# bowang-lab/BioReason

Hardware: AMD Instinct MI355X
Metric: GRPO samples/sec (NT-500M+Qwen3-1.7B, DNA 2x1024, prompt 2180, gen 256) (higher is better)
Workload: dtype bf16

## Files before the change

bioreason_amd/csrc/k_decgemm.hip:

```cpp
#include "bra_decgemm.h"
#include "bra_api_internal.h"

namespace bra {

#define BRA_DG2_HEAD_PARAMS const bf16_t* h_x, const bf16_t* h_W, const bf16_t* h_res, const float* h_ss_in, int h_ldx, int h_ldres, int h_M, int h_N, \
                            int h_K, int h_nss_in
#define BRA_DG2_HEAD_ARGS(g) (g).x, (g).W, (g).res, (g).ss_in, (int)(g).ldx, (int)(g).ldres, (g).M, (g).N, (g).K, (g).nss_in
template <int MODE, int NORM, int ACT, int OUTF32, int NW, int NL, int WIDE = 0, int PK = 0, int FAST = 0, int F8 = 0>
__global__ __launch_bounds__(NW * 64) void dec_gemm2_kernel(BRA_DG2_HEAD_PARAMS, DecGemm2Args g0) {
    DecGemm2Args g = g0;
    g.x = h_x; g.W = h_W; g.res = h_res; g.ss_in = h_ss_in; g.ldx = h_ldx; g.ldres = h_ldres; g.M = h_M; g.N = h_N; g.K = h_K; g.nss_in = h_nss_in;
    constexpr bool W32 = WIDE >= 2;
    static_assert(WIDE != 3 || (!FAST && NORM == 0), "32 rows, multi-round: not the fast form, no folded norm");
    static_assert(!WIDE || (MODE == 0 && NORM != 1), "wide rows: 16-column tiles, statistics applied in the epilogue");
    static_assert(!FAST || (PK && NORM != 1), "fast form: packed weights, folded norm or none");
    static_assert(!F8 || (FAST && NL % 2 == 0 && NW != 16 && !WIDE), "fp8 weights: fast form, two k-steps per 16-byte request");
    static_assert(WIDE != 2 || !F8, "32 rows: bf16 weights");
    constexpr int NLW = F8 ? NL / 2 : NL;
    constexpr int NH = W32 ? 2 : 1;
    constexpr int NBUF = (W32 && NW == 16) ? 1 : 2;
    __shared__ float red[NBUF][NH * NW][64][4];
    constexpr int KS = MODE ? 64 : 32;
    constexpr int NCOL = MODE ? 8 : 16;
    const int tid = (int)threadIdx.x, lane = tid & 63, wave = tid >> 6;
    const int fr = lane & 15, fq = lane >> 4;
    if (!FAST) dg2_stamp(g, 0);
    const int nsteps = FAST ? NW * NL : g.K / KS;
    const int ntiles = (g.N + NCOL - 1) / NCOL;
    const int lrow = MODE ? (fr & 7) : fr;
    const int koff = MODE ? ((fr >> 3) * 32 + fq * 8) : fq * 8;
    const int xr = lrow < g.M ? lrow : g.M - 1;
    const bf16_t* xp = FAST ? g.x + (dg2_mul24(xr, (int)g.ldx) + (unsigned)koff) : g.x + (long)xr * g.ldx + koff;
    auto x2_ptr = [&]() -> const bf16_t* {
        const int xr2 = lrow + 16 < g.M ? lrow + 16 : g.M - 1;
        return FAST ? g.x + (dg2_mul24(xr2, (int)g.ldx) + (unsigned)koff) : g.x + (long)xr2 * g.ldx + koff;
    };
    auto second_half = [&]() -> DecGemm2Args {
        DecGemm2Args g2 = g;
        g2.M = g.M - 16;
        if (g.res) g2.res = g.res + 16 * g.ldres;
        g2.out = OUTF32 ? (void*)((float*)g.out + 16 * g.ldo) : (void*)((bf16_t*)g.out + 16 * g.ldo);
        if (g.ss_out) g2.ss_out = g.ss_out + 16 * (long)g.nss_out;
        return g2;
    };
    const u32x4 zero4 = {0u, 0u, 0u, 0u};
    const int rounds = FAST ? 1 : (nsteps + NW * NL - 1) / (NW * NL);
    int tile = (int)blockIdx.x;
    int rn = tile * NCOL + lrow; rn = rn < g.N ? rn : g.N - 1;
    const bf16_t* wp = FAST ? g.W : g.W + (long)rn * g.ldw + koff;

    const int em = fr < g.M ? fr : g.M - 1;
    int en = tile * NCOL + 4 * fq; en = en + 3 < g.N ? en : (g.N >= 4 ? g.N - 4 : 0);
    u32x2 resv = {0u, 0u}, resv2 = {0u, 0u};
    if (!FAST && !ACT && !OUTF32 && g.res) resv = ld8(g.res + (long)em * g.ldres + en);
    auto em2_row = [&]() -> int { return fr + 16 < g.M ? fr : g.M - 17; };

    const int per = NORM ? g.nss_in >> 3 : 0;
    f32x4 pv[8];
    __shared__ float rs_lds[W32 ? 32 : (WIDE ? 16 : 8)];
    if (NORM == 1) {
        const float* pp = g.ss_in + (long)(lane >> 3) * g.nss_in + (lane & 7) * per;
#pragma unroll
        for (int i = 0; i < 8; ++i) pv[i] = *reinterpret_cast<const f32x4*>(pp + (4 * i < per ? 4 * i : 0));
    }
    float rstd = 1.f;

    if (WIDE != 3 && rounds == 1) {
        int st[NL];
#pragma unroll
        for (int u = 0; u < NL; ++u)
            st[u] = PK ? wave * NL + u
                             : (MODE ? wave + NW * u : 2 * (wave + NW * (u >> 1)) + (u & 1));
        long so[NL];
#pragma unroll
        for (int u = 0; u < NL; ++u) so[u] = FAST ? (long)(u * KS) : (long)(st[u] < nsteps ? st[u] : nsteps - 1) * KS;
        if (FAST) xp += (unsigned)(wave * (NL * KS));
        constexpr bool X2LATE = W32 && NW == 16;
        u32x4 w0[NLW], w1[NLW], x[NL], nv[NL], x2[(W32 && !X2LATE) ? NL : 1];
        f32x4 sc0 = {1.f, 1.f, 1.f, 1.f}, sc1 = sc0;
#pragma unroll
        for (int u = 0; u < NL; ++u) x[u] = ld16(xp + so[u]);
        if (NORM == 1) {
#pragma unroll
            for (int u = 0; u < NL; ++u) nv[u] = ld16(g.nw + koff + so[u]);
        }
        long wo[NLW];
#pragma unroll
        for (int u = 0; u < NLW; ++u) wo[u] = FAST ? (long)(u * 512) : (PK ? (long)(st[u] < nsteps ? st[u] : nsteps - 1) * 512 : so[u]);
        const unsigned wlane = (unsigned)(wave * (NLW * 512) + lane * 8);
        auto scale_of = [&](int t) -> f32x4 {
            return *reinterpret_cast<const f32x4*>(g.wscale + (unsigned)(t * NCOL + ((4 * fq) & (NCOL - 1))));
        };
        auto tile_base = [&](int t) -> const bf16_t* {
            if (FAST) return g.W + (long)t * (NW * NLW * 512) + wlane;
            if (PK) return g.W + (long)t * nsteps * 512 + lane * 8;
            int rnn = t * NCOL + lrow; rnn = rnn < g.N ? rnn : g.N - 1;
            return g.W + (long)rnn * g.ldw + koff;
        };
        wp = tile_base(tile);
#pragma unroll
        for (int u = 0; u < NLW; ++u) {
            w0[u] = ld16_nt(wp + wo[u]);
            if (W32 && u == 0) sched_fence();
        }
        const bf16_t* xp2 = xp;
        if constexpr (W32) {
            sched_fence();
            xp2 = x2_ptr();
            if (FAST) xp2 += (unsigned)(wave * (NL * KS));
            if constexpr (!X2LATE) {
#pragma unroll
                for (int u = 0; u < NL; ++u) x2[u] = ld16(xp2 + so[u]);
            }
            if (!FAST && !ACT && !OUTF32 && g.res) resv2 = ld8(g.res + (long)(em2_row() + 16) * g.ldres + en);
        }
        if (F8) {
            sched_fence();
            sc0 = scale_of(tile);
        }
        if (FAST && !ACT && !OUTF32) {
            const bf16_t* rp = g.res ? g.res : g.x;
            const unsigned ro = g.res ? dg2_mul24(em, (int)g.ldres) + (unsigned)en : 0u;
            resv = ld8(rp + ro);
            if (W32) resv2 = ld8(rp + (g.res ? dg2_mul24(em2_row() + 16, (int)g.ldres) + (unsigned)en : 0u));
        }
        sched_fence();
        if (!FAST) dg2_stamp(g, 1);
        constexpr int NPASS = WIDE == 1 ? 2 : 1;
        f32x4 sq[NPASS][8];
        const int swave = W32 ? 4 : 1, sbase = W32 ? 8 * wave : 0;
        if (NORM == 2 && wave < swave) {
#pragma unroll
            for (int pass = 0; pass < NPASS; ++pass) {
                const int srow = (lane >> 3) + 8 * pass + sbase;
                const int sr = srow < g.M ? srow : g.M - 1;
                const float* pp = FAST ? g.ss_in + (dg2_mul24(sr, g.nss_in) + (unsigned)((lane & 7) * per))
                                       : g.ss_in + (long)sr * g.nss_in + (lane & 7) * per;
#pragma unroll
                for (int i = 0; i < 8; ++i) sq[pass][i] = *reinterpret_cast<const f32x4*>(pp + (4 * i < per ? 4 * i : 0));
            }
#pragma unroll
            for (int pass = 0; pass < NPASS; ++pass)
#pragma unroll
                for (int i = 0; i < 8; ++i) reg_fence(sq[pass][i]);
        }
        auto fold_stats = [&]() {
#pragma unroll
            for (int pass = 0; pass < NPASS; ++pass) {
                const int srow = (lane >> 3) + 8 * pass + sbase;
                const float rs = dg2_fold_rstd(sq[pass], per, g.inv_K, g.eps);
                if ((lane & 7) == 0) rs_lds[srow] = rs;
            }
        };
        if (NORM == 1) {
#pragma unroll
            for (int i = 0; i < 8; ++i) reg_fence(pv[i]);
            float s = 0.f;
#pragma unroll
            for (int i = 0; i < 8; ++i) s += 4 * i < per ? (pv[i][0] + pv[i][1]) + (pv[i][2] + pv[i][3]) : 0.f;
            s += wave_shfl_xor(s, 1); s += wave_shfl_xor(s, 2); s += wave_shfl_xor(s, 4);
            rstd = rsqrtf(wave_shfl(s, xr * 8) / (float)g.K + g.eps);
#pragma unroll
            for (int u = 0; u < NL; ++u) {
                float xf[8], nf[8];
                unpack8(x[u], xf); unpack8(nv[u], nf);
#pragma unroll
                for (int i = 0; i < 8; ++i) xf[i] = nf[i] * round_bf(xf[i] * rstd);
                x[u] = pack8(xf);
            }
        }
#pragma unroll
        for (int u = 0; u < NL; ++u) if (!FAST && st[u] >= nsteps) x[u] = zero4;
        if constexpr (W32 && !X2LATE) {
#pragma unroll
            for (int u = 0; u < NL; ++u) if (!FAST && st[u] >= nsteps) x2[u] = zero4;
        }
        const int G = (int)gridDim.x;
        const int nmine = (ntiles - tile + G - 1) / G;
        auto issue = [&](u32x4 (&wn)[NLW], f32x4& scn, int t) {
            const bf16_t* wpn = tile_base(t);
#pragma unroll
            for (int u = 0; u < NLW; ++u) wn[u] = ld16_nt(wpn + wo[u]);
            if (F8) scn = scale_of(t);
        };
        auto compute = [&](u32x4 (&wc)[NLW], const f32x4& scc, int t, int it) {
            f32x4 acc = {0.f, 0.f, 0.f, 0.f};
            if constexpr (F8 != 0) {
#pragma unroll
                for (int u = 0; u < NLW; ++u) {
                    acc = mfma_16x16x32(f8x8_to_bf16x8(wc[u].x, wc[u].y), x[2 * u], acc);
                    acc = mfma_16x16x32(f8x8_to_bf16x8(wc[u].z, wc[u].w), x[2 * u + 1], acc);
                }
            } else {
#pragma unroll
                for (int u = 0; u < NL; ++u) acc = mfma_16x16x32(wc[u], x[u], acc);
            }
            f32x4 acc2 = {0.f, 0.f, 0.f, 0.f};
            if constexpr (X2LATE) {
                sched_fence();
#pragma unroll
                for (int u = 0; u < NL; ++u) x[u] = ld16(xp2 + so[u]);
#pragma unroll
                for (int u = 0; u < NL; ++u) if (!FAST && st[u] >= nsteps) x[u] = zero4;
#pragma unroll
                for (int u = 0; u < NL; ++u) acc2 = mfma_16x16x32(wc[u], x[u], acc2);
            } else if constexpr (W32) {
#pragma unroll
                for (int u = 0; u < NL; ++u) acc2 = mfma_16x16x32(wc[u], x2[u], acc2);
            }
            if (NORM == 2 && it == 0 && wave < swave) fold_stats();
            float (*slab)[64][4] = red[NBUF == 2 ? it & 1 : 0];
#pragma unroll
            for (int r = 0; r < 4; ++r) slab[wave][lane][r] = acc[r];
            if constexpr (W32) {
#pragma unroll
                for (int r = 0; r < 4; ++r) slab[NW + wave][lane][r] = acc2[r];
            }
            if (!FAST && it == 0) dg2_stamp(g, 2);
            __syncthreads();
            if (!FAST && it == 0) dg2_stamp(g, 3);
            if (wave == it % NW) {
                float v[4];
                dg2_reduce<NW>(slab, lane, v);
                if (NORM == 2) {
                    const int mrow = MODE ? (fr & 7) : fr;
                    const float rsf = rs_lds[mrow < g.M ? mrow : g.M - 1];
#pragma unroll
                    for (int r = 0; r < 4; ++r) v[r] *= rsf;
                }
                if (F8) {
#pragma unroll
                    for (int r = 0; r < 4; ++r) v[r] *= scc[r];
                }
                dg2_epilogue<MODE, ACT, OUTF32, PK>(g, v, t, lane, it == 0, resv);
            }
            if constexpr (W32) {
                if (wave == (it + 1) % NW) {
                    float v[4];
                    dg2_reduce<NW>(slab + NW, lane, v);
                    if (NORM == 2) {
                        const float rsf = rs_lds[16 + em2_row()];
#pragma unroll
                        for (int r = 0; r < 4; ++r) v[r] *= rsf;
                    }
                    const DecGemm2Args g2 = second_half();
                    dg2_epilogue<MODE, ACT, OUTF32, PK>(g2, v, t, lane, it == 0, resv2);
                }
            }
            if (!FAST && it == 0) dg2_stamp(g, 4);
        };
        if (NW == 16) {
            compute(w0, sc0, tile, 0);
            return;
        }
        int it = 0;
        for (; it + 2 < nmine; it += 2) {
            issue(w1, sc1, tile + (it + 1) * G); compute(w0, sc0, tile + it * G, it);
            issue(w0, sc0, tile + (it + 2) * G); compute(w1, sc1, tile + (it + 1) * G, it + 1);
        }
        if (nmine - it == 2) {
            issue(w1, sc1, tile + (it + 1) * G); compute(w0, sc0, tile + it * G, it);
            compute(w1, sc1, tile + (it + 1) * G, it + 1);
        } else {
            compute(w0, sc0, tile + it * G, it);
        }
        return;
    }

    if constexpr (WIDE == 2) return;
    constexpr bool X2LATE_MR = W32 && NW == 16;
    for (int it = 0; tile < ntiles; ++it, tile += (int)gridDim.x) {
        rn = tile * NCOL + lrow; rn = rn < g.N ? rn : g.N - 1;
        wp = g.W + (long)rn * g.ldw + koff;
        f32x4 acc = {0.f, 0.f, 0.f, 0.f}, acc2 = acc;
        for (int rd = 0; rd < rounds; ++rd) {
            const int base = rd * NW * NL;
            int st[NL];
#pragma unroll
            for (int u = 0; u < NL; ++u) st[u] = base + (MODE ? wave + NW * u : 2 * (wave + NW * (u >> 1)) + (u & 1));
            u32x4 w[NL], x[NL], nv[NL], x2[(W32 && !X2LATE_MR) ? NL : 1];
            const bf16_t* wpk = g.W + ((long)tile * nsteps * 64 + lane) * 8;
#pragma unroll
            for (int u = 0; u < NL; ++u) {
                const int sc = st[u] < nsteps ? st[u] : nsteps - 1;
                w[u] = PK ? ld16_nt(wpk + (long)sc * 512) : ld16_nt(wp + (long)sc * KS);
            }
#pragma unroll
            for (int u = 0; u < NL; ++u) { const int sc = st[u] < nsteps ? st[u] : nsteps - 1; x[u] = ld16(xp + (long)sc * KS); }
            const bf16_t* xp2 = xp;
            if constexpr (W32) {
                sched_fence();
                xp2 = x2_ptr();
                if (it == 0 && rd == 0 && !ACT && !OUTF32 && g.res) resv2 = ld8(g.res + (long)(em2_row() + 16) * g.ldres + en);
                if constexpr (!X2LATE_MR) {
#pragma unroll
                    for (int u = 0; u < NL; ++u) { const int sc = st[u] < nsteps ? st[u] : nsteps - 1; x2[u] = ld16(xp2 + (long)sc * KS); }
                }
            }
            if (NORM == 1) {
#pragma unroll
                for (int u = 0; u < NL; ++u) { const int sc = st[u] < nsteps ? st[u] : nsteps - 1; nv[u] = ld16(g.nw + koff + (long)sc * KS); }
                if (it == 0 && rd == 0) {
                    float s = 0.f;
#pragma unroll
                    for (int i = 0; i < 8; ++i) s += 4 * i < per ? (pv[i][0] + pv[i][1]) + (pv[i][2] + pv[i][3]) : 0.f;
                    s += wave_shfl_xor(s, 1); s += wave_shfl_xor(s, 2); s += wave_shfl_xor(s, 4);
                    rstd = rsqrtf(wave_shfl(s, xr * 8) / (float)g.K + g.eps);
                }
#pragma unroll
                for (int u = 0; u < NL; ++u) {
                    float xf[8], nf[8];
                    unpack8(x[u], xf); unpack8(nv[u], nf);
#pragma unroll
                    for (int i = 0; i < 8; ++i) xf[i] = nf[i] * round_bf(xf[i] * rstd);
                    x[u] = pack8(xf);
                }
            }
#pragma unroll
            for (int u = 0; u < NL; ++u) acc = mfma_16x16x32(st[u] < nsteps ? w[u] : zero4, x[u], acc);
            if constexpr (X2LATE_MR) {
                sched_fence();
#pragma unroll
                for (int u = 0; u < NL; ++u) { const int sc = st[u] < nsteps ? st[u] : nsteps - 1; x[u] = ld16(xp2 + (long)sc * KS); }
#pragma unroll
                for (int u = 0; u < NL; ++u) acc2 = mfma_16x16x32(st[u] < nsteps ? w[u] : zero4, x[u], acc2);
            } else if constexpr (W32) {
#pragma unroll
                for (int u = 0; u < NL; ++u) acc2 = mfma_16x16x32(st[u] < nsteps ? w[u] : zero4, x2[u], acc2);
            }
        }
        float (*slab)[64][4] = red[NBUF == 2 ? it & 1 : 0];
#pragma unroll
        for (int r = 0; r < 4; ++r) slab[wave][lane][r] = acc[r];
        if constexpr (W32) {
#pragma unroll
            for (int r = 0; r < 4; ++r) slab[NW + wave][lane][r] = acc2[r];
        }
        __syncthreads();
        if (wave == it % NW) {
            float v[4];
#pragma unroll
            for (int r = 0; r < 4; ++r) {
                float s = 0.f;
#pragma unroll
                for (int wv = 0; wv < NW; ++wv) s += slab[wv][lane][r];
                v[r] = s;
            }
            dg2_epilogue<MODE, ACT, OUTF32>(g, v, tile, lane, it == 0, resv);
        }
        if constexpr (W32) {
            if (wave == (it + 1) % NW) {
                float v[4];
#pragma unroll
                for (int r = 0; r < 4; ++r) {
                    float s = 0.f;
#pragma unroll
                    for (int wv = 0; wv < NW; ++wv) s += slab[NW + wv][lane][r];
                    v[r] = s;
                }
                const DecGemm2Args g2 = second_half();
                dg2_epilogue<MODE, ACT, OUTF32>(g2, v, tile, lane, it == 0, resv2);
            }
            if (NBUF == 1) __syncthreads();
        }
    }
}

__global__ __launch_bounds__(256) void row_sumsq_kernel(const bf16_t* x, long ldx, int K, float* ss, int nss) {
    __shared__ float part[4];
    const int r = (int)blockIdx.x, tid = (int)threadIdx.x;
    float s = 0.f;
    for (int j = tid; j < K / 8; j += 256) {
        float f[8];
        unpack8(ld16(x + (long)r * ldx + j * 8), f);
#pragma unroll
        for (int i = 0; i < 8; ++i) s += f[i] * f[i];
    }
    s = wave_sum<64>(s);
    if ((tid & 63) == 0) part[tid >> 6] = s;
    __syncthreads();
    for (int j = tid; j < nss; j += 256) ss[(long)r * nss + j] = j == 0 ? (part[0] + part[1]) + (part[2] + part[3]) : 0.f;
}

template <int MODE>
__global__ __launch_bounds__(256) void dec_pack_kernel(const bf16_t* W, long ldw, int N, int K, const bf16_t* nw, bf16_t* out) {
    constexpr int KS = MODE ? 64 : 32, NCOL = MODE ? 8 : 16;
    const int nsteps = K / KS;
    const long nchunk = (long)(N / NCOL) * nsteps * 64;
    const long c = (long)blockIdx.x * 256 + threadIdx.x;
    if (c >= nchunk) return;
    const int lane = (int)(c & 63);
    const long ts = c >> 6;
    const int step = (int)(ts % nsteps), tile = (int)(ts / nsteps);
    const int fr = lane & 15, fq = lane >> 4;
    const int row = tile * NCOL + (MODE ? (fr & 7) : fr);
    const int col = step * KS + (MODE ? ((fr >> 3) * 32 + fq * 8) : fq * 8);
    u32x4 v = ld16(W + (long)row * ldw + col);
    if (nw) {
        float f[8], s[8];
        unpack8(v, f); unpack8(ld16(nw + col), s);
#pragma unroll
        for (int i = 0; i < 8; ++i) f[i] *= s[i];
        v = pack8(f);
    }
    st16(out + c * 8, v);
}

__global__ __launch_bounds__(256) void dec_rowscale_fp8_kernel(const bf16_t* W, long ldw, int N, int K, const bf16_t* nw, float* scale) {
    const int row = (int)blockIdx.x * 4 + ((int)threadIdx.x >> 6), lane = (int)threadIdx.x & 63;
    if (row >= N) return;
    float mx = 0.f;
    for (int j = lane; j < K / 8; j += 64) {
        float f[8], s[8];
        unpack8(ld16(W + (long)row * ldw + j * 8), f);
        if (nw) { unpack8(ld16(nw + j * 8), s);
#pragma unroll
            for (int i = 0; i < 8; ++i) f[i] *= s[i]; }
#pragma unroll
        for (int i = 0; i < 8; ++i) mx = fmaxf(mx, fabsf(f[i]));
    }
    for (int m = 32; m >= 1; m >>= 1) mx = fmaxf(mx, wave_shfl_xor(mx, m));
    if (lane == 0) scale[row] = mx > 0.f ? mx * (1.0f / 448.0f) : 1.0f;
}

template <int MODE>
__global__ __launch_bounds__(256) void dec_pack_fp8_kernel(const bf16_t* W, long ldw, int N, int K, const bf16_t* nw, const float* scale,
                                                           unsigned* out) {
    constexpr int KS = MODE ? 64 : 32, NCOL = MODE ? 8 : 16;
    const int npair = K / KS / 2;
    const long nchunk = (long)(N / NCOL) * npair * 64;
    const long c = (long)blockIdx.x * 256 + threadIdx.x;
    if (c >= nchunk) return;
    const int lane = (int)(c & 63);
    const long ts = c >> 6;
    const int s2 = (int)(ts % npair), tile = (int)(ts / npair);
    const int fr = lane & 15, fq = lane >> 4;
    const int row = tile * NCOL + (MODE ? (fr & 7) : fr);
    const float inv = 1.0f / scale[row];
    unsigned o[4];
#pragma unroll
    for (int h = 0; h < 2; ++h) {
        const int col = (2 * s2 + h) * KS + (MODE ? ((fr >> 3) * 32 + fq * 8) : fq * 8);
        float f[8];
        unpack8(ld16(W + (long)row * ldw + col), f);
        if (nw) { float s[8]; unpack8(ld16(nw + col), s);
#pragma unroll
            for (int i = 0; i < 8; ++i) f[i] *= s[i]; }
        unsigned b[8];
#pragma unroll
        for (int i = 0; i < 8; ++i) b[i] = f32_to_e4m3(f[i] * inv);
        o[2 * h] = b[0] | (b[1] << 8) | (b[2] << 16) | (b[3] << 24);
        o[2 * h + 1] = b[4] | (b[5] << 8) | (b[6] << 16) | (b[7] << 24);
    }
    u32x4 v = {o[0], o[1], o[2], o[3]};
    *reinterpret_cast<u32x4*>(out + c * 4) = v;
}

static void dg2_waves_and_chunks(int nsteps, bool wide, int& nw, int& nl) {
    nw = (wide && nsteps >= 128) ? 16 : (nsteps >= 64 ? 8 : 4);
    const int spw = (nsteps + nw - 1) / nw;
    nl = (spw >= 12 && spw % 12 == 0) ? 12 : ((spw == 10 && nw == 8) ? 10 : (spw > 4 ? 8 : 4));
}

template <int MODE, int NORM, int ACT, int OUTF32, int WIDE = 0>
static int launch_dg2(const DecGemm2Args& g, bra_stream_t st) {
    constexpr int KS = MODE ? 64 : 32;
    const int nsteps = g.K / KS;
    int nw, nl;
    dg2_waves_and_chunks(nsteps, WIDE != 0, nw, nl);
    if (NORM == 2 && (nsteps + nw * nl - 1) / (nw * nl) != 1) return BRA_ERR_UNSUPPORTED;
    const int ntiles = MODE ? g.N / 8 : (g.N + 15) / 16;
    const int gmax = nw == 16 ? ntiles : (nw >= 8 ? 256 : 512);
    const dim3 grid(ntiles < gmax ? ntiles : gmax);
    constexpr long ROWS = WIDE == 2 ? 32 : 16;
    const bool fits32 = g.ldx < (1 << 24) && g.ldres < (1 << 24) && ROWS * g.ldx < (1L << 30) && ROWS * g.ldres + g.N < (1L << 30) &&
                        ROWS * g.nss_in < (1L << 24);
#ifdef BRA_DEBUG
    const bool probed = g.probe != nullptr;
#else
    const bool probed = false;
#endif
    const bool fast = NORM != 1 && (g.packed & 1) && nsteps == nw * nl && !probed && fits32;
    (void)fast;
#define BRA_DG2(NW_, NL_)                                                                                                      \
    do {                                                                                                                       \
        if constexpr (NORM != 1 && !WIDE && NW_ != 16 && NL_ % 2 == 0) {                                                       \
            if (g.wscale) {                                                                                                    \
                if (!fast) return BRA_ERR_UNSUPPORTED;                                                                         \
                BRA_LAUNCH((dec_gemm2_kernel<MODE, NORM, ACT, OUTF32, NW_, NL_, WIDE, 1, 1, 1>), grid, dim3(NW_ * 64), 0, st, BRA_DG2_HEAD_ARGS(g), g); \
                break;                                                                                                         \
            }                                                                                                                  \
        }                                                                                                                      \
        if (g.wscale) return BRA_ERR_UNSUPPORTED;                                                                              \
         \
        if constexpr (NORM != 1 && !(WIDE == 2 && NORM == 2 && NW_ == 16 && NL_ == 12)) {                                      \
            if (fast) {                                                                                                        \
                BRA_LAUNCH((dec_gemm2_kernel<MODE, NORM, ACT, OUTF32, NW_, NL_, WIDE, 1, 1>), grid, dim3(NW_ * 64), 0, st, BRA_DG2_HEAD_ARGS(g), g); \
                break;                                                                                                         \
            }                                                                                                                  \
        }                                                                                                                      \
        if constexpr (WIDE == 2) {                                                                                             \
                                                                      \
            if (nsteps > NW_ * NL_) {                                                                                          \
                 \
                if constexpr (NORM == 0 && (NW_ < 16 || NL_ == 8)) {                                                           \
                    if (g.packed & 1) {                                                                                        \
                        BRA_LAUNCH((dec_gemm2_kernel<MODE, NORM, ACT, OUTF32, NW_, NL_, 3, 1>), grid, dim3(NW_ * 64), 0, st, BRA_DG2_HEAD_ARGS(g), g); \
                        break;                                                                                                 \
                    }                                                                                                          \
                    if constexpr (NW_ < 16) {                                                                                  \
                        BRA_LAUNCH((dec_gemm2_kernel<MODE, NORM, ACT, OUTF32, NW_, NL_, 3, 0>), grid, dim3(NW_ * 64), 0, st, BRA_DG2_HEAD_ARGS(g), g); \
                        break;                                                                                                 \
                    }                                                                                                          \
                }                                                                                                              \
                return BRA_ERR_UNSUPPORTED;                                                                                    \
            }                                                                                                                  \
            if constexpr (NW_ * NL_ > 64) return BRA_ERR_UNSUPPORTED;                                                          \
        }                                                                                                                      \
        if constexpr (!(WIDE == 2 && NW_ * NL_ > 64)) {                                                                        \
            if (g.packed & 1) BRA_LAUNCH((dec_gemm2_kernel<MODE, NORM, ACT, OUTF32, NW_, NL_, WIDE, 1>), grid, dim3(NW_ * 64), 0, st, BRA_DG2_HEAD_ARGS(g), g); \
            else BRA_LAUNCH((dec_gemm2_kernel<MODE, NORM, ACT, OUTF32, NW_, NL_, WIDE, 0>), grid, dim3(NW_ * 64), 0, st, BRA_DG2_HEAD_ARGS(g), g);  \
        }                                                                                                                      \
    } while (0)
    if (nw == 16) {
        if constexpr (WIDE != 0) { if (nl == 12) BRA_DG2(16, 12); else if (nl == 8) BRA_DG2(16, 8); else BRA_DG2(16, 4); }
    }
    else if (nw == 8) { if (nl == 12) BRA_DG2(8, 12); else if (nl == 10) BRA_DG2(8, 10); else if (nl == 8) BRA_DG2(8, 8); else BRA_DG2(8, 4); }
    else { if (nl == 12) BRA_DG2(4, 12); else if (nl == 8) BRA_DG2(4, 8); else BRA_DG2(4, 4); }
#undef BRA_DG2
    return BRA_LAUNCH_STATUS();
}

}

using namespace bra;

static int dec_gemm2_any(const void* x, long ldx, const float* ss_in, int nss_in, const void* norm_w, float eps,
                        const void* W, long ldw, const void* res, long ldres, void* out, long ldo, float* ss_out,
                        int nss_out, int M, int N, int K, int act, int out_f32, int packed, void* probe, void* stream,
                        const float* wscale = nullptr);

extern "C" int bra_dec_gemm2(const void* x, long ldx, const float* ss_in, int nss_in, const void* norm_w, float eps,
                             const void* W, long ldw, const void* res, long ldres, void* out, long ldo, float* ss_out,
                             int nss_out, int M, int N, int K, int act, int out_f32, void* stream) {
    return dec_gemm2_any(x, ldx, ss_in, nss_in, norm_w, eps, W, ldw, res, ldres, out, ldo, ss_out, nss_out, M, N, K, act, out_f32,
                         0, nullptr, stream);
}

extern "C" int bra_dec_gemm2_packed(const void* x, long ldx, const float* ss_in, int nss_in, const void* norm_w, float eps,
                                    const void* W, long ldw, const void* res, long ldres, void* out, long ldo, float* ss_out,
                                    int nss_out, int M, int N, int K, int act, int out_f32, int packed, void* stream) {
    return dec_gemm2_any(x, ldx, ss_in, nss_in, norm_w, eps, W, ldw, res, ldres, out, ldo, ss_out, nss_out, M, N, K, act, out_f32,
                         packed, nullptr, stream);
}

extern "C" int bra_dec_gemm2_fp8(const void* x, long ldx, const float* ss_in, int nss_in, float eps, const void* Wq, const float* wscale,
                                 const void* res, long ldres, void* out, long ldo, float* ss_out, int nss_out, int M, int N, int K,
                                 int act, int out_f32, int norm_folded, void* stream) {
    if (!Wq || !wscale) return BRA_ERR_ARG;
    return dec_gemm2_any(x, ldx, norm_folded ? ss_in : nullptr, norm_folded ? nss_in : 0, norm_folded ? Wq : nullptr, eps, Wq, K, res, ldres,
                         out, ldo, ss_out, nss_out, M, N, K, act, out_f32, norm_folded ? 3 : 1, nullptr, stream, wscale);
}

#ifdef BRA_DEBUG
extern "C" int bra_dec_gemm2_probe(const void* x, long ldx, const float* ss_in, int nss_in, const void* norm_w, float eps,
                                   const void* W, long ldw, const void* res, long ldres, void* out, long ldo, float* ss_out,
                                   int nss_out, int M, int N, int K, int act, int out_f32, int packed, void* probe, void* stream) {
    return dec_gemm2_any(x, ldx, ss_in, nss_in, norm_w, eps, W, ldw, res, ldres, out, ldo, ss_out, nss_out, M, N, K, act, out_f32,
                         packed, probe, stream);
}
#endif

static int dec_gemm2_any(const void* x, long ldx, const float* ss_in, int nss_in, const void* norm_w, float eps,
                        const void* W, long ldw, const void* res, long ldres, void* out, long ldo, float* ss_out,
                        int nss_out, int M, int N, int K, int act, int out_f32, int packed, void* probe, void* stream,
                        const float* wscale) {
    (void)probe;
    if (wscale && (M > 8 || !(packed & 1) || (norm_w && !(packed & 2)))) return BRA_ERR_UNSUPPORTED;
    if (M <= 0 || M > 32 || N <= 0 || K <= 0 || K % 32 || ldx % 8 || ldw % 8 || !x || !W || !out) return BRA_ERR_ARG;
    if (act && (N % 16 || out_f32 || res || ss_out)) return BRA_ERR_ARG;
    if (out_f32 && res) return BRA_ERR_ARG;
    if (norm_w && (!ss_in || nss_in < 32 || nss_in % 32 || nss_in > 256)) return BRA_ERR_ARG;
    if (res && ldres % 4) return BRA_ERR_ARG;
    const bool wide = M > 8;
    const bool diag = !wide && !act && !out_f32 && N % 8 == 0 && K % 64 == 0 && (N + 15) / 16 < 256 && N / 8 <= 256;
    if (ss_out && nss_out < (diag ? N / 8 : (N + 15) / 16)) return BRA_ERR_ARG;
    DecGemm2Args g = {(const bf16_t*)x, ldx, ss_in, nss_in, (const bf16_t*)norm_w, eps, (const bf16_t*)W, ldw,
                      (const bf16_t*)res, ldres, out, ldo, ss_out, nss_out, M, N, K, packed, wscale, BRA_DBG_INIT((unsigned long long*)probe) 1.f / (float)K};
    if (packed && (N % (diag ? 8 : 16) || K % (diag ? 64 : 32))) return BRA_ERR_ARG;
    bra_stream_t st = (bra_stream_t)stream;
    if ((packed & 2) && !(packed & 1)) return BRA_ERR_ARG;
    if (M > 16) {
        if (norm_w && !(packed & 2)) return BRA_ERR_UNSUPPORTED;
        if (norm_w) {
            if (act) return launch_dg2<0, 2, 1, 0, 2>(g, st);
            if (out_f32) return launch_dg2<0, 2, 0, 1, 2>(g, st);
            return launch_dg2<0, 2, 0, 0, 2>(g, st);
        }
        if (act) return launch_dg2<0, 0, 1, 0, 2>(g, st);
        if (out_f32) return launch_dg2<0, 0, 0, 1, 2>(g, st);
        return launch_dg2<0, 0, 0, 0, 2>(g, st);
    }
    if (wide) {
        if (norm_w && !(packed & 2)) return BRA_ERR_UNSUPPORTED;
        if (norm_w) {
            if (act) return launch_dg2<0, 2, 1, 0, 1>(g, st);
            if (out_f32) return launch_dg2<0, 2, 0, 1, 1>(g, st);
            return launch_dg2<0, 2, 0, 0, 1>(g, st);
        }
        if (act) return launch_dg2<0, 0, 1, 0, 1>(g, st);
        if (out_f32) return launch_dg2<0, 0, 0, 1, 1>(g, st);
        return launch_dg2<0, 0, 0, 0, 1>(g, st);
    }
    if (norm_w && (packed & 2)) {
        if (act) return launch_dg2<0, 2, 1, 0>(g, st);
        if (out_f32) return launch_dg2<0, 2, 0, 1>(g, st);
        return diag ? launch_dg2<1, 2, 0, 0>(g, st) : launch_dg2<0, 2, 0, 0>(g, st);
    }
    if (norm_w) {
        if (act) return launch_dg2<0, 1, 1, 0>(g, st);
        if (out_f32) return launch_dg2<0, 1, 0, 1>(g, st);
        return diag ? launch_dg2<1, 1, 0, 0>(g, st) : launch_dg2<0, 1, 0, 0>(g, st);
    }
    if (act) return launch_dg2<0, 0, 1, 0>(g, st);
    if (out_f32) return launch_dg2<0, 0, 0, 1>(g, st);
    return diag ? launch_dg2<1, 0, 0, 0>(g, st) : launch_dg2<0, 0, 0, 0>(g, st);
}

extern "C" int bra_dec_pack_weights_rows(const void* W, long ldw, int N, int K, int act, int out_f32, const void* norm_w, int rows,
                                         void* out, void* stream);
extern "C" int bra_dec_pack_weights(const void* W, long ldw, int N, int K, int act, int out_f32, const void* norm_w, void* out,
                                    void* stream) {
    return bra_dec_pack_weights_rows(W, ldw, N, K, act, out_f32, norm_w, 8, out, stream);
}

extern "C" int bra_dec_pack_weights_rows(const void* W, long ldw, int N, int K, int act, int out_f32, const void* norm_w, int rows,
                                         void* out, void* stream) {
    if (!W || !out || N <= 0 || K <= 0 || ldw % 8 || rows <= 0 || rows > 16) return BRA_ERR_ARG;
    const bool diag = rows <= 8 && !act && !out_f32 && N % 8 == 0 && K % 64 == 0 && (N + 15) / 16 < 256 && N / 8 <= 256;
    if (N % (diag ? 8 : 16) || K % (diag ? 64 : 32)) return BRA_ERR_UNSUPPORTED;
    const long nchunk = (long)N * K / 8;
    const dim3 grid((unsigned)((nchunk + 255) / 256));
    if (diag) BRA_LAUNCH((dec_pack_kernel<1>), grid, dim3(256), 0, (bra_stream_t)stream, (const bf16_t*)W, ldw, N, K, (const bf16_t*)norm_w, (bf16_t*)out);
    else BRA_LAUNCH((dec_pack_kernel<0>), grid, dim3(256), 0, (bra_stream_t)stream, (const bf16_t*)W, ldw, N, K, (const bf16_t*)norm_w, (bf16_t*)out);
    return BRA_LAUNCH_STATUS();
}

extern "C" int bra_dec_pack_weights_fp8(const void* W, long ldw, int N, int K, int act, int out_f32, const void* norm_w, void* out_q,
                                        float* out_scale, void* stream) {
    if (!W || !out_q || !out_scale || N <= 0 || K <= 0 || ldw % 8) return BRA_ERR_ARG;
    const bool diag = !act && !out_f32 && N % 8 == 0 && K % 64 == 0 && (N + 15) / 16 < 256 && N / 8 <= 256;
    if (N % (diag ? 8 : 16) || K % (diag ? 128 : 64)) return BRA_ERR_UNSUPPORTED;
    {
        int nw, nl;
        const int nsteps = K / (diag ? 64 : 32);
        dg2_waves_and_chunks(nsteps, false, nw, nl);
        if (nsteps != nw * nl || nl % 2 || nw == 16) return BRA_ERR_UNSUPPORTED;
    }
    bra_stream_t st = (bra_stream_t)stream;
    BRA_LAUNCH(dec_rowscale_fp8_kernel, dim3((N + 3) / 4), dim3(256), 0, st, (const bf16_t*)W, ldw, N, K, (const bf16_t*)norm_w, out_scale);
    int rc = BRA_LAUNCH_STATUS();
    if (rc) return rc;
    const long nchunk = (long)N * K / 16;
    const dim3 grid((unsigned)((nchunk + 255) / 256));
    if (diag) BRA_LAUNCH((dec_pack_fp8_kernel<1>), grid, dim3(256), 0, st, (const bf16_t*)W, ldw, N, K, (const bf16_t*)norm_w, out_scale, (unsigned*)out_q);
    else BRA_LAUNCH((dec_pack_fp8_kernel<0>), grid, dim3(256), 0, st, (const bf16_t*)W, ldw, N, K, (const bf16_t*)norm_w, out_scale, (unsigned*)out_q);
    return BRA_LAUNCH_STATUS();
}

extern "C" int bra_row_sumsq(const void* x, long ldx, int M, int K, float* ss, int nss, void* stream) {
    if (M <= 0 || M > 32 || K <= 0 || K % 8 || ldx % 8 || !x || !ss || nss < 1) return BRA_ERR_ARG;
    BRA_LAUNCH(row_sumsq_kernel, dim3(M), dim3(256), 0, (bra_stream_t)stream, (const bf16_t*)x, ldx, K, ss, nss);
    return BRA_LAUNCH_STATUS();
}
```

include/bioreason_hip_debug.h:

```cpp
#ifndef BIOREASON_HIP_DEBUG_H
#define BIOREASON_HIP_DEBUG_H
#include "bioreason_hip.h"
#ifdef __cplusplus
extern "C" {
#endif

int bra_gemm_set_variant(int v);
int bra_gemm_set_ring_fill(int pct);
int bra_gemm_set_row_split(int on);
int bra_gemm_set_epi_lds(int on);
int bra_sample_set_one_launch(int on);
int bra_gemm_set_glds_rows(int rows);
int bra_attn_set_block_order(int legacy);
int bra_attn_set_fwd4(int on);
int bra_attn_set_bwd4(int mask);
int bra_attn_set_probe(void* buf);


int bra_dec_gemm2_probe(const void* x, long ldx, const float* ss_in, int nss_in, const void* norm_w, float eps, const void* W,
                        long ldw, const void* res, long ldres, void* out, long ldo, float* ss_out, int nss_out, int M, int N,
                        int K, int act, int out_f32, int packed, void* probe, void* stream);
int bra_debug_set_probe(void* p);

int bra_gridsync_bytes(void);
int bra_persist_layer_desc_size(void);
int bra_persist_set_stamps(void* p);
int bra_qwen_layers_persist(const void* layers_dev, int L, int R, int copies, int H, int Hq, int Hkv, int hd, int F, int P,
                            long vt_pitch, int C, long cp, float eps, float scale, const float* cosT, const float* sinT,
                            const int* pos, const float* rope_rows, const void* pmask, int t, const int* t_dev, void* x,
                            void* qkv, void* o, void* h, void* act, float* ss_ws, int nss, float* part_o, float* part_ml,
                            int nslot, void* sync, int prefetch, int stop_after, int timeout_us, void* stream);
int bra_qwen_decode_step_persist(const void* layers_host, const void* layers_dev, int L, int R, int copies, int H, int Hq, int Hkv,
                                 int hd, int F, int P, long vt_pitch, int C, long cp, int V, float eps, float scale, const void* E,
                                 const void* norm_w, const float* cosT, const float* sinT, const int* tok, const int* pos,
                                 const void* pmask, int t, const int* t_dev, int embed_done, void* x, void* qkv, void* o, void* h,
                                 void* act, float* ss_ws, int nss, float* part_o, float* part_ml, int nslot, float* logits,
                                 void* sync, int prefetch, int stop_after, int timeout_us, void* stream);
int bra_chain_probe(void* done, void* buf, void* errs, const void* wts, long wts_bytes, int nwg, int n, int chained, int wchunks,
                    int timeout_us, void* stream_a, void* stream_b);
int bra_gridbar_probe(void* sync, void* buf, void* errs, const void* wts, long wts_bytes, int nwg, int iters, int mode,
                      int wchunks, int timeout_us, void* stream);

#ifdef __cplusplus
}
#endif
#endif
```

Before: 19.73.

## Add three-deep weight prefetch ring to decode GEMM for act/f32-out forms

Adds a depth-3 weight buffering variant of the decode GEMM kernel for 8-wave, 8-chunk, folded-norm forms with activation or fp32 output. When a block owns three or fewer tiles, all weight sets are loaded up front. With six or more tiles per block, a rotating ring refills each buffer right after its MFMA work. The aim is to keep more weight bytes in flight so HBM latency is hidden during memory-bound decode. The cost is extra register pressure, plus new debug switches to force depth 2 or cap the grid.

```diff
diff --git a/bioreason_amd/csrc/k_decgemm.hip b/bioreason_amd/csrc/k_decgemm.hip
--- a/bioreason_amd/csrc/k_decgemm.hip
+++ b/bioreason_amd/csrc/k_decgemm.hip
@@ -8,6 +8,8 @@
 #define BRA_DG2_HEAD_ARGS(g) (g).x, (g).W, (g).res, (g).ss_in, (int)(g).ldx, (int)(g).ldres, (g).M, (g).N, (g).K, (g).nss_in
 template <int MODE, int NORM, int ACT, int OUTF32, int NW, int NL, int WIDE = 0, int PK = 0, int FAST = 0, int F8 = 0>
 __global__ __launch_bounds__(NW * 64) void dec_gemm2_kernel(BRA_DG2_HEAD_PARAMS, DecGemm2Args g0) {
+    constexpr int DEPTH = FAST >= 2 ? 3 : 2;
+    constexpr bool RING = FAST == 2;
     DecGemm2Args g = g0;
     g.x = h_x; g.W = h_W; g.res = h_res; g.ss_in = h_ss_in; g.ldx = h_ldx; g.ldres = h_ldres; g.M = h_M; g.N = h_N; g.K = h_K; g.nss_in = h_nss_in;
     constexpr bool W32 = WIDE >= 2;
@@ -16,6 +18,7 @@
     static_assert(!FAST || (PK && NORM != 1), "fast form: packed weights, folded norm or none");
     static_assert(!F8 || (FAST && NL % 2 == 0 && NW != 16 && !WIDE), "fp8 weights: fast form, two k-steps per 16-byte request");
     static_assert(WIDE != 2 || !F8, "32 rows: bf16 weights");
+    static_assert(FAST == 0 || FAST == 1 || ((FAST == 2 || FAST == 3) && !WIDE && NW != 16), "three weight sets: fast 8-row forms of 4 or 8 waves");
     constexpr int NLW = F8 ? NL / 2 : NL;
     constexpr int NH = W32 ? 2 : 1;
     constexpr int NBUF = (W32 && NW == 16) ? 1 : 2;
@@ -76,8 +79,8 @@
         for (int u = 0; u < NL; ++u) so[u] = FAST ? (long)(u * KS) : (long)(st[u] < nsteps ? st[u] : nsteps - 1) * KS;
         if (FAST) xp += (unsigned)(wave * (NL * KS));
         constexpr bool X2LATE = W32 && NW == 16;
-        u32x4 w0[NLW], w1[NLW], x[NL], nv[NL], x2[(W32 && !X2LATE) ? NL : 1];
-        f32x4 sc0 = {1.f, 1.f, 1.f, 1.f}, sc1 = sc0;
+        u32x4 w0[NLW], w1[NLW], w2[DEPTH == 3 ? NLW : 1], x[NL], nv[NL], x2[(W32 && !X2LATE) ? NL : 1];
+        f32x4 sc0 = {1.f, 1.f, 1.f, 1.f}, sc1 = sc0, sc2 = sc0;
 #pragma unroll
         for (int u = 0; u < NL; ++u) x[u] = ld16(xp + so[u]);
         if (NORM == 1) {
@@ -100,6 +103,7 @@
         wp = tile_base(tile);
 #pragma unroll
         for (int u = 0; u < NLW; ++u) {
+            if (DEPTH == 3 && !F8 && u >= 4) { w0[u] = ld16_nt((g.W + ((long)tile * (NW * NLW * 512) + (u >> 2) * 2048)) + (wlane + (unsigned)((u & 3) * 512))); continue; }
             w0[u] = ld16_nt(wp + wo[u]);
             if (W32 && u == 0) sched_fence();
         }
@@ -144,6 +148,19 @@
 #pragma unroll
                 for (int i = 0; i < 8; ++i) reg_fence(sq[pass][i]);
         }
+        if constexpr (DEPTH == 3) {
+            const int G0 = (int)gridDim.x;
+            const int t1 = tile + G0 < ntiles ? tile + G0 : tile;
+            const int t2 = tile + 2 * G0 < ntiles ? tile + 2 * G0 : t1;
+            const bf16_t* wq = tile_base(t1);
+#pragma unroll
+            for (int u = 0; u < NLW; ++u) w1[u] = ld16_nt(wq + wo[u]);
+            wq = tile_base(t2);
+#pragma unroll
+            for (int u = 0; u < NLW; ++u) w2[u] = ld16_nt(wq + wo[u]);
+            if (F8) { sc1 = scale_of(t1); sc2 = scale_of(t2); }
+            sched_fence();
+        }
         auto fold_stats = [&]() {
 #pragma unroll
             for (int pass = 0; pass < NPASS; ++pass) {
@@ -183,7 +200,7 @@
             for (int u = 0; u < NLW; ++u) wn[u] = ld16_nt(wpn + wo[u]);
             if (F8) scn = scale_of(t);
         };
-        auto compute = [&](u32x4 (&wc)[NLW], const f32x4& scc, int t, int it) {
+        auto compute = [&](u32x4 (&wc)[NLW], f32x4& scc, int t, int it, bool refill = false) {
             f32x4 acc = {0.f, 0.f, 0.f, 0.f};
             if constexpr (F8 != 0) {
 #pragma unroll
@@ -208,7 +225,11 @@
 #pragma unroll
                 for (int u = 0; u < NL; ++u) acc2 = mfma_16x16x32(wc[u], x2[u], acc2);
             }
-            if (NORM == 2 && it == 0 && wave < swave) fold_stats();
+            const f32x4 scv = scc;
+            if constexpr (DEPTH == 3) {
+                if (refill) { sched_fence(); issue(wc, scc, t + 3 * G); }
+            }
+            if (!(DEPTH == 3 && RING) && NORM == 2 && it == 0 && wave < swave) fold_stats();
             float (*slab)[64][4] = red[NBUF == 2 ? it & 1 : 0];
 #pragma unroll
             for (int r = 0; r < 4; ++r) slab[wave][lane][r] = acc[r];
@@ -230,7 +251,7 @@
                 }
                 if (F8) {
 #pragma unroll
-                    for (int r = 0; r < 4; ++r) v[r] *= scc[r];
+                    for (int r = 0; r < 4; ++r) v[r] *= scv[r];
                 }
                 dg2_epilogue<MODE, ACT, OUTF32, PK>(g, v, t, lane, it == 0, resv);
             }
@@ -254,6 +275,41 @@
             return;
         }
         int it = 0;
+        if constexpr (DEPTH == 3 && !RING) {
+            compute(w0, sc0, tile, 0);
+            if (nmine >= 2) compute(w1, sc1, tile + G, 1);
+            if (nmine >= 3) compute(w2, sc2, tile + 2 * G, 2);
+            return;
+        }
+        if constexpr (DEPTH == 3) {
+            if (NORM == 2 && wave < swave) fold_stats();
+            auto tl = [&](int i) { return tile + i * G; };
+            do {
+                compute(w0, sc0, tl(it), it, true);
+                compute(w1, sc1, tl(it + 1), it + 1, true);
+                compute(w2, sc2, tl(it + 2), it + 2, true);
+                it += 3;
+            } while (it + 6 <= nmine);
+            const int rem = nmine - it;
+            if (rem == 3) {
+                compute(w0, sc0, tl(it), it);
+                compute(w1, sc1, tl(it + 1), it + 1);
+                compute(w2, sc2, tl(it + 2), it + 2);
+                return;
+            }
+            compute(w0, sc0, tl(it), it, true);
+            if (rem == 4) {
+                compute(w1, sc1, tl(it + 1), it + 1);
+                compute(w2, sc2, tl(it + 2), it + 2);
+                compute(w0, sc0, tl(it + 3), it + 3);
+            } else {
+                compute(w1, sc1, tl(it + 1), it + 1, true);
+                compute(w2, sc2, tl(it + 2), it + 2);
+                compute(w0, sc0, tl(it + 3), it + 3);
+                compute(w1, sc1, tl(it + 4), it + 4);
+            }
+            return;
+        }
         for (; it + 2 < nmine; it += 2) {
             issue(w1, sc1, tile + (it + 1) * G); compute(w0, sc0, tile + it * G, it);
             issue(w0, sc0, tile + (it + 2) * G); compute(w1, sc1, tile + (it + 1) * G, it + 1);
@@ -462,6 +518,11 @@
     nl = (spw >= 12 && spw % 12 == 0) ? 12 : ((spw == 10 && nw == 8) ? 10 : (spw > 4 ? 8 : 4));
 }
 
+template <int MODE, int NORM, int ACT, int OUTF32, int WIDE, int NW, int NL>
+constexpr bool dg2_depth3_form = MODE == 0 && NORM == 2 && (ACT || OUTF32) && WIDE == 0 && NW == 8 && NL == 8;
+static int g_dg2_depth2 = 0;
+static int g_dg2_grid_cap = 0;
+
 template <int MODE, int NORM, int ACT, int OUTF32, int WIDE = 0>
 static int launch_dg2(const DecGemm2Args& g, bra_stream_t st) {
     constexpr int KS = MODE ? 64 : 32;
@@ -470,7 +531,8 @@
     dg2_waves_and_chunks(nsteps, WIDE != 0, nw, nl);
     if (NORM == 2 && (nsteps + nw * nl - 1) / (nw * nl) != 1) return BRA_ERR_UNSUPPORTED;
     const int ntiles = MODE ? g.N / 8 : (g.N + 15) / 16;
-    const int gmax = nw == 16 ? ntiles : (nw >= 8 ? 256 : 512);
+    int gmax = nw == 16 ? ntiles : (nw >= 8 ? 256 : 512);
+    if (nw != 16 && g_dg2_grid_cap > 0 && g_dg2_grid_cap < gmax) gmax = g_dg2_grid_cap;
     const dim3 grid(ntiles < gmax ? ntiles : gmax);
     constexpr long ROWS = WIDE == 2 ? 32 : 16;
     const bool fits32 = g.ldx < (1 << 24) && g.ldres < (1 << 24) && ROWS * g.ldx < (1L << 30) && ROWS * g.ldres + g.N < (1L << 30) &&
@@ -493,6 +555,16 @@
         }                                                                                                                      \
         if (g.wscale) return BRA_ERR_UNSUPPORTED;                                                                              \
          \
+        if constexpr (dg2_depth3_form<MODE, NORM, ACT, OUTF32, WIDE, NW_, NL_>) {                                              \
+            if (fast && !g_dg2_depth2 && (ntiles + (int)grid.x - 1) / (int)grid.x <= 3) {                                     \
+                BRA_LAUNCH((dec_gemm2_kernel<MODE, NORM, ACT, OUTF32, NW_, NL_, 0, 1, 3>), grid, dim3(NW_ * 64), 0, st, BRA_DG2_HEAD_ARGS(g), g); \
+                break;                                                                                                         \
+            }                                                                                                                  \
+            if (fast && !g_dg2_depth2 && ntiles / (int)grid.x >= 6) {                                                          \
+                BRA_LAUNCH((dec_gemm2_kernel<MODE, NORM, ACT, OUTF32, NW_, NL_, 0, 1, 2>), grid, dim3(NW_ * 64), 0, st, BRA_DG2_HEAD_ARGS(g), g); \
+                break;                                                                                                         \
+            }                                                                                                                  \
+        }                                                                                                                      \
         if constexpr (NORM != 1 && !(WIDE == 2 && NORM == 2 && NW_ == 16 && NL_ == 12)) {                                      \
             if (fast) {                                                                                                        \
                 BRA_LAUNCH((dec_gemm2_kernel<MODE, NORM, ACT, OUTF32, NW_, NL_, WIDE, 1, 1>), grid, dim3(NW_ * 64), 0, st, BRA_DG2_HEAD_ARGS(g), g); \
@@ -569,6 +641,8 @@
     return dec_gemm2_any(x, ldx, ss_in, nss_in, norm_w, eps, W, ldw, res, ldres, out, ldo, ss_out, nss_out, M, N, K, act, out_f32,
                          packed, probe, stream);
 }
+extern "C" int bra_dec_gemm2_set_depth2(int on) { g_dg2_depth2 = on; return 0; }
+extern "C" int bra_dec_gemm2_set_grid_cap(int cap) { g_dg2_grid_cap = cap > 0 ? cap : 0; return 0; }
 #endif
 
 static int dec_gemm2_any(const void* x, long ldx, const float* ss_in, int nss_in, const void* norm_w, float eps,
diff --git a/include/bioreason_hip_debug.h b/include/bioreason_hip_debug.h
--- a/include/bioreason_hip_debug.h
+++ b/include/bioreason_hip_debug.h
@@ -20,6 +20,8 @@
 int bra_dec_gemm2_probe(const void* x, long ldx, const float* ss_in, int nss_in, const void* norm_w, float eps, const void* W,
                         long ldw, const void* res, long ldres, void* out, long ldo, float* ss_out, int nss_out, int M, int N,
                         int K, int act, int out_f32, int packed, void* probe, void* stream);
+int bra_dec_gemm2_set_depth2(int on);
+int bra_dec_gemm2_set_grid_cap(int cap);
 int bra_debug_set_probe(void* p);
 
 int bra_gridsync_bytes(void);
```

New measurement: 19.64. About the same (-0.5%).
